# RohanVKashyap/resolution-pde

Measured on AMD Instinct MI355X. Metric: training samples/sec, FFNO2D NS 256^2, higher is better.
Workload: dtype f32; 1 GPU; FFNO2D(1,1,width=64,n_layers=4,n_modes=20,factor=4,ff_weight_norm,n_ff_layers=3,layer_norm,dropout=0.1) train step on [B,1,256,256] Gaussian random fields (BASELINE configs[2]); batch_per_gpu=32, global_batch=32, optimizer=AdamW lr=1e-3 (rpde.optim.FlatAdamW: torch.optim.AdamW's rule, one kernel), parallelism=single, grad_bucket_bytes=6828576, target=input advanced by a fixed spectral filter (utils/synthetic.py:advance)

## Files before the change

resolution-pde_amd/csrc/ff_bwd_split.hip:

```cpp
#include "ff_bwd_split.h"
#include "ff_fused.h"
#include "h2.h"
#include "pointwise.h"
#include "wgrad_h2.h"

namespace rpde {

constexpr int FS_WAVES = 8;
constexpr int FS_MAX_GRID = 256;
struct FsA {
  const float* g; const float* z3; const float* d2;
  float* dz3; float* du2; float* dzb;
  const char* wimg; const float* consts;
  const float* gamma; const float* beta;
  float* part;
  long P; int layer_norm; float eps; int post_act;
  DropCfg drop2;
  int ntiles;
};

constexpr int FA_DZBUF = 0;
constexpr int FA_VEC = FA_DZBUF + 16384;
constexpr int FA_ACC = FA_VEC + 512;
constexpr int FA_INFO = FA_ACC + 7168;
constexpr int FA_LDS = FA_INFO + 256;

__global__ __launch_bounds__(64 * FS_WAVES, 2) void k_ffs_adjoint(const FsA A0) {
  __shared__ __attribute__((aligned(16))) char smem[FA_LDS];
  FsA A = A0;
  A.drop2 = drop_resolve(A0.drop2);
  const int tid = threadIdx.x, l = tid & 63, w = tid >> 6, g = l >> 4, li = l & 15;
  f16x8 w3h[2][2], w3l[2][2];
  {
    const char* base = A.wimg + (long)w * FF3_WAVE_IMG + l * 16;
#pragma unroll
    for (int f = 0; f < 4; ++f) {
      w3h[f >> 1][f & 1] = *reinterpret_cast<const f16x8*>(base + f * 2048);
      w3l[f >> 1][f & 1] = *reinterpret_cast<const f16x8*>(base + f * 2048 + 1024);
    }
    float* vecw = reinterpret_cast<float*>(smem + FA_VEC);
    float* accw = reinterpret_cast<float*>(smem + FA_ACC);
    for (int i = tid; i < 128; i += 64 * FS_WAVES) vecw[i] = i < 64 ? (A.gamma ? A.gamma[i] : 1.f) : (A.beta ? A.beta[i - 64] : 0.f);
    for (int i = tid; i < 1792; i += 64 * FS_WAVES) accw[i] = 0.f;
  }
  const float* const vec = reinterpret_cast<const float*>(smem + FA_VEC);
  float* const acc_db2 = reinterpret_cast<float*>(smem + FA_ACC);
  float* const acc_db3 = acc_db2 + 256;
  float* const acc_dg = acc_db2 + 768;
  float* const acc_dbt = acc_db2 + 1280;
  float* const info = reinterpret_cast<float*>(smem + FA_INFO);
  const float winv3 = A.consts[2];
  const int q3 = l >> 4, feat = 4 * li;

  float4 g4n = make_float4(0.f, 0.f, 0.f, 0.f), z4n = g4n, d2n[4];
  auto issue = [&](int tile) {
    const long p = min((long)tile * 32 + 4 * w + q3, A.P - 1);
    g4n = *reinterpret_cast<const float4*>(A.g + p * 64 + feat);
    z4n = *reinterpret_cast<const float4*>(A.z3 + p * 64 + feat);
#pragma unroll
    for (int blk = 0; blk < 2; ++blk)
#pragma unroll
      for (int t = 0; t < 2; ++t)
        d2n[blk * 2 + t] = *reinterpret_cast<const float4*>(A.d2 + min((long)tile * 32 + 16 * blk + li, A.P - 1) * 256 + 16 * (2 * w + t) + 4 * g);
  };
#pragma unroll
  for (int i = 0; i < 4; ++i) d2n[i] = make_float4(0.f, 0.f, 0.f, 0.f);
  if ((int)blockIdx.x < A.ntiles) issue(blockIdx.x);
  lds_barrier();

  int par = 0;
  for (int tile = blockIdx.x; tile < A.ntiles; tile += gridDim.x, par ^= 1) {
    const int next_tile = tile + gridDim.x;
    const long p0 = (long)tile * 32;
    const int ptl = 4 * w + q3;
    const long pt3 = p0 + ptl;
    const bool live3 = pt3 < A.P;
    const long off3 = min(pt3, A.P - 1) * 64 + feat;
    const float4 g4 = g4n, z4 = z4n;
    float4 dq[4];
#pragma unroll
    for (int i = 0; i < 4; ++i) dq[i] = d2n[i];
    if (next_tile < A.ntiles) issue(next_tile);

    float s4[4] = {1.f, 1.f, 1.f, 1.f};
    if (A.drop2.on()) drop_scale4(A.drop2, (uint64_t)(pt3 * 64 + feat), s4);
    const float tz[4] = {z4.x * s4[0], z4.y * s4[1], z4.z * s4[2], z4.w * s4[3]};
    float gy[4] = {g4.x, g4.y, g4.z, g4.w};
    if (!live3) { gy[0] = gy[1] = gy[2] = gy[3] = 0.f; }
    float dz[4], dzb;
    float dgm[4] = {0.f, 0.f, 0.f, 0.f}, dbt[4] = {0.f, 0.f, 0.f, 0.f};
    if (A.layer_norm) {
      const float mean = row_all16<false>((tz[0] + tz[1]) + (tz[2] + tz[3])) * (1.f / 64.f);
      const float m2 = row_all16<false>((tz[0] - mean) * (tz[0] - mean) + (tz[1] - mean) * (tz[1] - mean) +
                                        (tz[2] - mean) * (tz[2] - mean) + (tz[3] - mean) * (tz[3] - mean));
      const float rstd = rsqrtf(m2 * (1.f / 64.f) + A.eps);
      const float4 gm = *reinterpret_cast<const float4*>(vec + feat);
      const float4 bt = *reinterpret_cast<const float4*>(vec + 64 + feat);
      const float gmv[4] = {gm.x, gm.y, gm.z, gm.w}, btv[4] = {bt.x, bt.y, bt.z, bt.w};
      float xh[4], dxh[4], s1 = 0.f, s2 = 0.f, am = 0.f;
#pragma unroll
      for (int k = 0; k < 4; ++k) {
        xh[k] = (tz[k] - mean) * rstd;
        float dy = gy[k];
        if (A.post_act) dy *= dact_f(A.post_act, xh[k] * gmv[k] + btv[k]);
        dgm[k] = dy * xh[k];
        dbt[k] = dy;
        dxh[k] = dy * gmv[k];
        s1 += dxh[k];
        s2 += dxh[k] * xh[k];
        am = fmaxf(am, fabsf(dxh[k]));
      }
      const float S1 = row_all16<false>(s1) * (1.f / 64.f), S2 = row_all16<false>(s2) * (1.f / 64.f);
      const float AM = row_all16<true>(am);
#pragma unroll
      for (int k = 0; k < 4; ++k) dz[k] = rstd * (dxh[k] - S1 - xh[k] * S2) * s4[k];
      dzb = rstd * (AM + fabsf(S1) + 8.f * fabsf(S2)) * A.drop2.scale;
    } else {
      float am = 0.f;
#pragma unroll
      for (int k = 0; k < 4; ++k) { dz[k] = gy[k] * dact_f(A.post_act, tz[k]) * s4[k]; am = fmaxf(am, fabsf(dz[k])); }
      dzb = row_all16<true>(am);
    }
    if (live3) *reinterpret_cast<float4*>(A.dz3 + off3) = make_float4(dz[0], dz[1], dz[2], dz[3]);
    {
      float b[4];
#pragma unroll
      for (int k = 0; k < 4; ++k) {
        b[k] = live3 ? dz[k] : 0.f;
        b[k] += lane_xor16(b[k]); b[k] += lane_xor32(b[k]);
        if (A.layer_norm) {
          dgm[k] += lane_xor16(dgm[k]); dgm[k] += lane_xor32(dgm[k]);
          dbt[k] += lane_xor16(dbt[k]); dbt[k] += lane_xor32(dbt[k]);
        }
      }
      if (q3 == 0) {
        float4* a3 = reinterpret_cast<float4*>(acc_db3 + w * 64 + feat);
        float4 v3 = *a3;
        v3.x += b[0]; v3.y += b[1]; v3.z += b[2]; v3.w += b[3];
        *a3 = v3;
        if (A.layer_norm) {
          float4* ag = reinterpret_cast<float4*>(acc_dg + w * 64 + feat);
          float4* ab = reinterpret_cast<float4*>(acc_dbt + w * 64 + feat);
          float4 vg = *ag, vb = *ab;
          vg.x += dgm[0]; vg.y += dgm[1]; vg.z += dgm[2]; vg.w += dgm[3];
          vb.x += dbt[0]; vb.y += dbt[1]; vb.z += dbt[2]; vb.w += dbt[3];
          *ag = vg;
          *ab = vb;
        }
      }
    }
    {
      float sdz, sdzi;
      h2_scale(dzb, 0, sdz, sdzi);
      uint2 hi, lo;
      h2_split4(dz[0] * sdz, dz[1] * sdz, dz[2] * sdz, dz[3] * sdz, hi, lo);
      const int ksz = li >> 3, cz = li & 3;
      char* dst = smem + FA_DZBUF + par * 8192 + (((ptl >> 4) * 2 + ksz) * 2) * 1024 + (cz * 16 + ((ptl & 15) ^ cz ^ (4 * ksz))) * 16 +
                  ((li >> 2) & 1) * 8;
      *reinterpret_cast<uint2*>(dst) = hi;
      *reinterpret_cast<uint2*>(dst + 1024) = lo;
      if (li == 0) {
        info[par * 32 + ptl] = dzb;
        if (live3) A.dzb[pt3] = dzb;
      }
    }
    lds_barrier();

    float bsum[8] = {0.f, 0.f, 0.f, 0.f, 0.f, 0.f, 0.f, 0.f};
#pragma unroll
    for (int blk = 0; blk < 2; ++blk) {
      const int zu = (l & 48) | ((l & 15) ^ (l >> 4));
      const char* zb = smem + FA_DZBUF + par * 8192 + (blk * 2) * 2048;
      const f16x8 zh0 = *reinterpret_cast<const f16x8*>(zb + zu * 16), zl0 = *reinterpret_cast<const f16x8*>(zb + 1024 + zu * 16);
      const f16x8 zh1 = *reinterpret_cast<const f16x8*>(zb + 2048 + (zu ^ 4) * 16), zl1 = *reinterpret_cast<const f16x8*>(zb + 3072 + (zu ^ 4) * 16);
      const long pt = p0 + 16 * blk + li;
      float sz, inv_a;
      h2_scale(info[par * 32 + blk * 16 + li], 0, sz, inv_a);
      inv_a *= winv3;
#pragma unroll
      for (int t = 0; t < 2; ++t) {
        f32x4v acc = {0.f, 0.f, 0.f, 0.f};
        acc = h2_mfma32(w3h[t][0], w3l[t][0], zh0, zl0, acc);
        acc = h2_mfma32(w3h[t][1], w3l[t][1], zh1, zl1, acc);
        const int hid = 16 * (2 * w + t) + 4 * g;
        const float4 d = dq[blk * 2 + t];
        float u[4] = {acc[0] * inv_a * d.x, acc[1] * inv_a * d.y, acc[2] * inv_a * d.z, acc[3] * inv_a * d.w};
#pragma unroll
        for (int r = 0; r < 4; ++r) pin(u[r]);
        if (pt < A.P) {
          *reinterpret_cast<float4*>(A.du2 + pt * 256 + hid) = make_float4(u[0], u[1], u[2], u[3]);
#pragma unroll
          for (int r = 0; r < 4; ++r) bsum[4 * t + r] += u[r];
        }
      }
    }
#pragma unroll
    for (int i = 0; i < 8; ++i) bsum[i] = row_sum15(bsum[i]);
    if (li == 15) {
#pragma unroll
      for (int i = 0; i < 8; ++i) acc_db2[16 * (2 * w + (i >> 2)) + 4 * g + (i & 3)] += bsum[i];
    }
  }
  lds_barrier();
  {
    float* part = A.part + (long)blockIdx.x * FF3_PART;
    for (int i = 256 + tid; i < FF3_PART; i += 64 * FS_WAVES) {
      float v;
      if (i < 512) v = acc_db2[i - 256];
      else {
        const float* a8 = acc_db3 + ((i - 512) >> 6) * 512 + ((i - 512) & 63);
        v = 0.f;
#pragma unroll
        for (int ww = 0; ww < FS_WAVES; ++ww) v += a8[ww * 64];
      }
      part[i] = v;
    }
  }
}

struct FsB {
  const float* du2; const float* d1; const float* x; const float* dzb; const float* w1;
  float* gx; float* slabs; float* part;
  const char* wimg; const float* consts;
  long P; float dmax; int ntiles;
};

constexpr int FL_PANEL = 8192;
constexpr int FL_DUBUF = 0;
constexpr int FL_PAN = FL_DUBUF + 32768;
constexpr int FL_X = FL_PAN + 4 * FL_PANEL;
constexpr int FL_W1 = FL_X + FL_PANEL;
constexpr int FL_LDS = FL_W1 + 65536;

__global__ __launch_bounds__(64 * FS_WAVES, 2) void k_ffs_layer1(const FsB A) {
  __shared__ __attribute__((aligned(16))) char smem[FL_LDS];
  __shared__ int einfo[FS_WAVES];
  __shared__ float xmax[FS_WAVES];
  __shared__ float wmax[FS_WAVES];
  __shared__ float acc_db1[256];
  const int tid = threadIdx.x, l = tid & 63, w = tid >> 6, g = l >> 4, li = l & 15;
  f16x8 w2h[2][8], w2l[2][8];
  {
    const char* base = A.wimg + (long)w * FF3_WAVE_IMG + l * 16;
#pragma unroll
    for (int f = 0; f < 16; ++f) {
      w2h[f >> 3][f & 7] = *reinterpret_cast<const f16x8*>(base + (4 + f) * 2048);
      w2l[f >> 3][f & 7] = *reinterpret_cast<const f16x8*>(base + (4 + f) * 2048 + 1024);
    }
  }
  if (tid < 256) acc_db1[tid] = 0.f;
  char* const wfrag = smem + FL_W1;
  float w_inv = 1.f;
  {
    constexpr int NF = 8 * 4 * 64 / (64 * FS_WAVES);
    float wv[NF][8];
    float m = 0.f;
#pragma unroll
    for (int r = 0; r < NF; ++r) {
      const int c = tid + r * 64 * FS_WAVES, fl = c & 63, nt = (c >> 6) & 3, ks = c >> 8;
#pragma unroll
      for (int j = 0; j < 8; ++j) {
        wv[r][j] = A.w1[(long)(32 * ks + 8 * (fl >> 4) + j) * 64 + 16 * nt + (fl & 15)];
        m = fmaxf(m, fabsf(wv[r][j]));
      }
    }
    m = wave_max(m);
    if (l == 0) wmax[w] = m;
    __syncthreads();
    m = 0.f;
#pragma unroll
    for (int i = 0; i < FS_WAVES; ++i) m = fmaxf(m, wmax[i]);
    float w_scale;
    h2_scale(m, 0, w_scale, w_inv);
#pragma unroll
    for (int r = 0; r < NF; ++r) {
      const int c = tid + r * 64 * FS_WAVES, fl = c & 63, nt = (c >> 6) & 3, ks = c >> 8;
      uint2 h0, l0, h1, l1;
      h2_split4(wv[r][0] * w_scale, wv[r][1] * w_scale, wv[r][2] * w_scale, wv[r][3] * w_scale, h0, l0);
      h2_split4(wv[r][4] * w_scale, wv[r][5] * w_scale, wv[r][6] * w_scale, wv[r][7] * w_scale, h1, l1);
      char* d = wfrag + (ks * 4 + nt) * 2048 + fl * 16;
      *reinterpret_cast<uint4*>(d) = make_uint4(h0.x, h0.y, h1.x, h1.y);
      *reinterpret_cast<uint4*>(d + 1024) = make_uint4(l0.x, l0.y, l1.x, l1.y);
    }
  }
  const float winv2 = A.consts[1], c3t = A.consts[3];

  const int xrow = tid >> 4, xc = tid & 15;
  float4 du2r[4], d1r[4], xr;
  float bzr[2];
  const unsigned cb = 32 * w + 4 * g;
  auto load_du2 = [&](int tile) {
    const long t0 = (long)tile * 32;
    const int rmax = (int)min(31L, A.P - 1 - t0);
    const float* __restrict__ src = A.du2 + t0 * 256;
    const float* __restrict__ bz = A.dzb + t0;
#pragma unroll
    for (int blk = 0; blk < 2; ++blk) {
      const unsigned r = (unsigned)min(16 * blk + li, rmax);
      bzr[blk] = bz[r];
#pragma unroll
      for (int t = 0; t < 2; ++t) du2r[blk * 2 + t] = *reinterpret_cast<const float4*>(src + (r * 256u + cb + 16u * t));
    }
  };
  auto load_d1 = [&](int tile) {
    const long t0 = (long)tile * 32;
    const int rmax = (int)min(31L, A.P - 1 - t0);
    const float* __restrict__ src = A.d1 + t0 * 256;
#pragma unroll
    for (int blk = 0; blk < 2; ++blk) {
      const unsigned r = (unsigned)min(16 * blk + li, rmax);
#pragma unroll
      for (int t = 0; t < 2; ++t) d1r[blk * 2 + t] = *reinterpret_cast<const float4*>(src + (r * 256u + cb + 16u * t));
    }
  };
  auto load_x = [&](int tile) {
    const long t0 = (long)tile * 32;
    const float* __restrict__ src = A.x + t0 * 64;
    xr = t0 + xrow < A.P ? *reinterpret_cast<const float4*>(src + (unsigned)(xrow * 64 + 4 * xc)) : make_float4(0.f, 0.f, 0.f, 0.f);
  };

  const int wm = w >> 1, wn = w & 1;
  typedef s16x4v __attribute__((address_space(3))) * lds_tr;
  f32x4v gw[4][2];
#pragma unroll
  for (int i = 0; i < 4; ++i)
#pragma unroll
    for (int j = 0; j < 2; ++j) gw[i][j] = (f32x4v){0.f, 0.f, 0.f, 0.f};
  int ea_used[2] = {15, 15}, eb_used = 15;
  int e_run = 15, e_x = 15;
  const int dg_mt = w & 1, dg_nt = w >> 1;

  if ((int)blockIdx.x < A.ntiles) { load_du2(blockIdx.x); load_d1(blockIdx.x); load_x(blockIdx.x); }
  lds_barrier();

  for (int tile = blockIdx.x; tile < A.ntiles; tile += gridDim.x) {
    const int next_tile = tile + gridDim.x;
    const bool has_next = next_tile < A.ntiles;
    const long p0 = (long)tile * 32;
    float inv_b[2];
#pragma unroll
    for (int blk = 0; blk < 2; ++blk) {
      float s_du2, ai;
      h2_scale(c3t * bzr[blk] * A.dmax, 0, s_du2, ai);
      inv_b[blk] = ai * winv2;
      const float4 a = du2r[blk * 2], b = du2r[blk * 2 + 1];
      const float hv[8] = {a.x * s_du2, a.y * s_du2, a.z * s_du2, a.w * s_du2, b.x * s_du2, b.y * s_du2, b.z * s_du2, b.w * s_du2};
      h2_put_frag(smem + FL_DUBUF + ((blk * 8 + w) * 2) * 1024 + l * 16, hv);
    }
    {
      float m = fmaxf(fmaxf(fabsf(xr.x), fabsf(xr.y)), fmaxf(fabsf(xr.z), fabsf(xr.w)));
      m = wave_max(m);
      if (l == 0) xmax[w] = m;
    }
    lds_barrier();

    float u[4][4];
    float bsum[8] = {0.f, 0.f, 0.f, 0.f, 0.f, 0.f, 0.f, 0.f};
    {
      f32x4v acc[2][2];
#pragma unroll
      for (int blk = 0; blk < 2; ++blk) {
        acc[blk][0] = (f32x4v){0.f, 0.f, 0.f, 0.f}; acc[blk][1] = (f32x4v){0.f, 0.f, 0.f, 0.f};
#pragma unroll
        for (int kap = 0; kap < 8; ++kap) {
          const char* hb = smem + FL_DUBUF + ((blk * 8 + kap) * 2) * 1024 + l * 16;
          const f16x8 bh = *reinterpret_cast<const f16x8*>(hb), bl = *reinterpret_cast<const f16x8*>(hb + 1024);
          acc[blk][0] = h2_mfma32(w2h[0][kap], w2l[0][kap], bh, bl, acc[blk][0]);
          acc[blk][1] = h2_mfma32(w2h[1][kap], w2l[1][kap], bh, bl, acc[blk][1]);
        }
      }
#pragma unroll
      for (int blk = 0; blk < 2; ++blk) {
        const bool live = p0 + 16 * blk + li < A.P;
#pragma unroll
        for (int t = 0; t < 2; ++t) {
          const float4 d4 = d1r[blk * 2 + t];
          const float d[4] = {d4.x, d4.y, d4.z, d4.w};
          float* v = u[blk * 2 + t];
          float s[4];
#pragma unroll
          for (int r = 0; r < 4; ++r) { s[r] = acc[blk][t][r] * inv_b[blk]; v[r] = s[r] * d[r]; }
          if (live) {
#pragma unroll
            for (int r = 0; r < 4; ++r) bsum[4 * t + r] = __builtin_fmaf(s[r], d[r], bsum[4 * t + r]);
          } else {
            v[0] = v[1] = v[2] = v[3] = 0.f;
          }
        }
      }
    }
    if (has_next) { load_du2(next_tile); load_d1(next_tile); }
#pragma unroll
    for (int i = 0; i < 8; ++i) bsum[i] = row_sum15(bsum[i]);
    if (li == 15) {
#pragma unroll
      for (int i = 0; i < 8; ++i) acc_db1[16 * (2 * w + (i >> 2)) + 4 * g + (i & 3)] += bsum[i];
    }
    {
      float m = 0.f;
#pragma unroll
      for (int i = 0; i < 4; ++i) m = fmaxf(fmaxf(m, fmaxf(fabsf(u[i][0]), fabsf(u[i][1]))), fmaxf(fabsf(u[i][2]), fabsf(u[i][3])));
      m = wave_max(m);
      e_run = max(e_run, (int)(__float_as_uint(m) >> 23) & 0xff);
      e_run = min(e_run, 254);
      const float scale = __uint_as_float((unsigned)(268 - e_run) << 23);
      char* const dst = smem + FL_PAN + (w >> 1) * FL_PANEL;
#pragma unroll
      for (int blk = 0; blk < 2; ++blk)
#pragma unroll
        for (int t = 0; t < 2; ++t) {
          const float* v = u[blk * 2 + t];
          uint2 hi, lo;
          h2_split4(v[0] * scale, v[1] * scale, v[2] * scale, v[3] * scale, hi, lo);
          const int off = stage_off(16 * blk + li, (w & 1) * 8 + 4 * t + g);
          *reinterpret_cast<uint2*>(dst + off) = hi;
          *reinterpret_cast<uint2*>(dst + 4096 + off) = lo;
        }
      if (l == 0) einfo[w] = e_run;
    }
    {
      float m = 0.f;
#pragma unroll
      for (int i = 0; i < FS_WAVES; ++i) m = fmaxf(m, xmax[i]);
      e_x = max(e_x, (int)(__float_as_uint(m) >> 23) & 0xff);
      e_x = min(e_x, 254);
      const float scale = __uint_as_float((unsigned)(268 - e_x) << 23);
      uint2 hi, lo;
      h2_split4(xr.x * scale, xr.y * scale, xr.z * scale, xr.w * scale, hi, lo);
      const int off = stage_off(xrow, xc);
      *reinterpret_cast<uint2*>(smem + FL_X + off) = hi;
      *reinterpret_cast<uint2*>(smem + FL_X + 4096 + off) = lo;
    }
    if (has_next) load_x(next_tile);
    lds_barrier();

    int lc = l;
    asm volatile("" : "+v"(lc));
    const int gc = lc >> 4, lic = lc & 15;
    {
      const int q = lic >> 2, pp = lic & 3;
      const int tsw = ((q >> 1) & 1) | ((gc & 1) << 1);
      const int trow = (8 * gc + q) * 128 + pp * 8;
      auto frag = [&](const char* panel, int tile, f16x8& hi, f16x8& lo) {
        const char* t = panel + trow + ((tile ^ tsw) << 5);
        union { struct { s16x4v a, b; } h; f16x8 v; } uh, ul;
        uh.h.a = __builtin_amdgcn_ds_read_tr16_b64_v4i16((lds_tr)(t));
        uh.h.b = __builtin_amdgcn_ds_read_tr16_b64_v4i16((lds_tr)(t + 512));
        ul.h.a = __builtin_amdgcn_ds_read_tr16_b64_v4i16((lds_tr)(t + 4096));
        ul.h.b = __builtin_amdgcn_ds_read_tr16_b64_v4i16((lds_tr)(t + 4096 + 512));
        hi = uh.v; lo = ul.v;
      };
      const int eb = __builtin_amdgcn_readfirstlane(e_x);
#pragma unroll
      for (int k = 0; k < 2; ++k) {
        const int ea = __builtin_amdgcn_readfirstlane(einfo[2 * wm + k]);
        if (ea + eb != ea_used[k] + eb_used) {
          const int d = (ea_used[k] + eb_used) - (ea + eb);
          const float f = d > -126 ? __uint_as_float((unsigned)(127 + d) << 23) : 0.f;
#pragma unroll
          for (int j = 0; j < 2; ++j) { gw[2 * k][j] *= f; gw[2 * k + 1][j] *= f; }
        }
        ea_used[k] = ea;
      }
      eb_used = eb;
      f16x8 bh[2], bl[2];
#pragma unroll
      for (int j = 0; j < 2; ++j) frag(smem + FL_X, 2 * wn + j, bh[j], bl[j]);
#pragma unroll
      for (int i = 0; i < 4; ++i) {
        f16x8 ah, al;
        frag(smem + FL_PAN + wm * FL_PANEL, i, ah, al);
#pragma unroll
        for (int j = 0; j < 2; ++j) gw[i][j] = h2_mfma32(ah, al, bh[j], bl[j], gw[i][j]);
      }
    }
    {
      f32x4v tot = (f32x4v){0.f, 0.f, 0.f, 0.f};
      const int row = 16 * dg_mt + lic;
#pragma unroll
      for (int hp = 0; hp < 8; ++hp) {
        const char* pa_ = smem + FL_PAN + (hp >> 1) * FL_PANEL + stage_off(row, 2 * (4 * (hp & 1) + gc));
        const f16x8 ah = *reinterpret_cast<const f16x8*>(pa_), al = *reinterpret_cast<const f16x8*>(pa_ + 4096);
        const char* wb = wfrag + (hp * 4 + dg_nt) * 2048 + lc * 16;
        const f16x8 bh = *reinterpret_cast<const f16x8*>(wb), bl = *reinterpret_cast<const f16x8*>(wb + 1024);
        const f32x4v part = h2_mfma32(ah, al, bh, bl, (f32x4v){0.f, 0.f, 0.f, 0.f});
        const int ek = __builtin_amdgcn_readfirstlane(einfo[hp]);
        const float fk = __uint_as_float((unsigned)(ek - 14) << 23) * w_inv;
        tot += part * fk;
      }
      float t0 = tot[0], t1 = tot[1], t2 = tot[2], t3 = tot[3];
      quad_transpose(t0, t1, t2, t3);
      const int rq = 16 * dg_mt + 4 * gc + (lic & 3);
      if (p0 + rq < A.P) *reinterpret_cast<float4*>(A.gx + p0 * 64 + (unsigned)(rq * 64 + 16 * dg_nt + 4 * (lic >> 2))) = make_float4(t0, t1, t2, t3);
    }
  }

  const float fb = __uint_as_float((unsigned)(eb_used - 14) << 23);
  float* __restrict__ out = A.slabs + (long)blockIdx.x * 256 * 64;
  const unsigned o0 = (unsigned)((wm * 64 + 4 * g) * 64 + wn * 32 + li);
#pragma unroll
  for (int i = 0; i < 4; ++i) {
    const float fa = __uint_as_float((unsigned)(ea_used[i >> 1] - 14) << 23);
#pragma unroll
    for (int j = 0; j < 2; ++j)
#pragma unroll
      for (int r = 0; r < 4; ++r) out[o0 + (unsigned)((16 * i + r) * 64 + 16 * j)] = gw[i][j][r] * fa * fb;
  }
  lds_barrier();
  if (tid < 256) A.part[(long)blockIdx.x * FF3_PART + tid] = acc_db1[tid];
}

bool ff_bwd_split_ok(long P, int hid, int dim) { return !switch_off("RPDE_FF_BWD_SPLIT") && wgrad_h2_dgrad_ok(P, hid, dim); }

int ff_bwd_split_launch(const rpde_ff_params* p, const float* const* ds, const float* z_last, const float* grad_out,
                        const float* x, float* dz3, float* du2, float* dzb, float* gx, float* slabs, float* gw1, float* part,
                        int* grid_out, long P, void* fimg, hipStream_t st, FoldJobs* folds) {
  RPDE_CHECK_ARG(ff_bwd_split_ok(P, p->dim * p->factor, p->dim) && ds && ds[0] && ds[1] && gx && gw1 && slabs,
                 "ff_bwd_split: unsupported call");
  const char* img;
  const float* consts;
  RPDE_TRY(ff3_fused_bwd_prepare(p, fimg, &img, &consts, st));
  const int ntiles = (int)((P + 31) / 32);
  int cus;
  RPDE_HIP(cu_count(&cus));
  int grid = cus < FS_MAX_GRID ? cus : FS_MAX_GRID;
  if (ntiles < grid) grid = ntiles;
  const DropCfg drop2 = make_drop(p->dropout_p, layer_seed(p->seed, 2), p->seed_epoch);

  FsA a;
  memset(&a, 0, sizeof(a));
  a.g = grad_out; a.z3 = z_last; a.d2 = ds[1];
  a.dz3 = dz3; a.du2 = du2; a.dzb = dzb;
  a.wimg = img; a.consts = consts; a.gamma = p->ln_gamma; a.beta = p->ln_beta; a.part = part;
  a.P = P; a.layer_norm = p->layer_norm; a.eps = p->ln_eps; a.post_act = p->post_act;
  a.drop2 = drop2; a.ntiles = ntiles;
  hipLaunchKernelGGL(k_ffs_adjoint, dim3(grid), dim3(64 * FS_WAVES), 0, st, a);
  RPDE_LAUNCH_CHECK();

  FsB b;
  memset(&b, 0, sizeof(b));
  b.du2 = du2; b.d1 = ds[0]; b.x = x; b.dzb = dzb; b.w1 = p->weights[0];
  b.gx = gx; b.slabs = slabs; b.part = part;
  b.wimg = img; b.consts = consts;
  b.P = P; b.dmax = 1.13f * drop2.scale;
  b.ntiles = ntiles;
  hipLaunchKernelGGL(k_ffs_layer1, dim3(grid), dim3(64 * FS_WAVES), 0, st, b);
  RPDE_LAUNCH_CHECK();
  *grid_out = grid;
  const int hid = p->dim * p->factor;
  if (folds && folds->add(slabs, gw1, hid * p->dim, grid, (long)hid * p->dim)) return RPDE_OK;
  return reduce_slabs(slabs, gw1, (long)hid * p->dim, grid, (long)hid * p->dim, 1.f, 0, st);
}

}
```

Before: 1046 samples/s.

## Restructure FF layer-1 backward pipeline: deeper prefetch, parked W2 fragments, priority split

Reworks the k_ffs_layer1 tile loop so du2 is staged into LDS one tile ahead and fetched two tiles ahead, while d1 and the x maximum for the next tile are loaded at the end of the current iteration. Loads are clamped to the last tile, which removes the has_next branches. Part of the W2 low-half fragments is parked in extra LDS to reduce register pressure, and the dgrad loop double-buffers its LDS fragment reads. Upper waves get a raised scheduling priority. Optional timestamp instrumentation and a profiling script are added behind RPDE_STAMPS. The cost is more LDS, which may affect occupancy at two blocks per CU, plus some redundant clamped loads.

Measured after the change: 1058 samples/s, median of 6. 1.01x the previous value.

```diff
diff --git a/profiles/ffs_layer1_stamps.py b/profiles/ffs_layer1_stamps.py
--- /dev/null
+++ b/profiles/ffs_layer1_stamps.py
@@ -0,0 +1,40 @@
+#!/usr/bin/env python3
+import ctypes as C
+import os
+import sys
+
+REPO = os.path.dirname(os.path.dirname(os.path.abspath(__file__)))
+for p in (REPO, os.path.join(REPO, "resolution-pde_amd")):
+    sys.path.insert(0, p)
+import numpy as np
+import torch
+from rpde import _lib
+from models.custom_layer import FeedForward
+
+lib = _lib.load()
+torch.manual_seed(0)
+ff = FeedForward(64, 4, n_layers=3, layer_norm=True, dropout=0.1).to("cuda")
+x = torch.randn(32, 256, 256, 64, device="cuda").requires_grad_(True)
+res, g = torch.randn_like(x), torch.randn_like(x)
+for _ in range(3):
+    ff(x, residual=res).backward(g)
+torch.cuda.synchronize()
+buf = (C.c_ulonglong * (3 * 64))()
+lib.rpde_debug_ffl_stamps.argtypes = [C.c_void_p]
+_lib.check(lib.rpde_debug_ffl_stamps(buf), "stamps")
+t = np.array(buf, dtype=np.uint64).reshape(3, 8, 8).astype(np.int64)
+names = ["top", "barrier 1 passed", "products + scaling done", "panels written, x requested", "barrier 2 passed",
+         "next du2 staged + requested", "gW1 done", "gx done"]
+for wi, wn in enumerate(("wave 0", "wave 3", "wave 6")):
+    print(wn)
+    for ti in range(7):
+        row = t[wi, ti]
+        print("   tile", ti + 5, " ".join(f"{names[i]}:+{int(row[i] - row[0])}" for i in range(1, 8)),
+              f" | tile period {int(t[wi, ti + 1, 0] - row[0])}")
+per = (t[:, 1:, 0] - t[:, :-1, 0]).astype(np.float64)
+seg = np.diff(np.concatenate([t[:, :7, :], t[:, 1:, :1]], axis=2), axis=2).astype(np.float64)
+print("mean share of the tile period, waves 0 / 3 / 6:")
+for i in range(8):
+    what = f"{names[i]} -> {names[i + 1] if i < 7 else 'x maximum, next top'}"
+    print(f"   {what:64s}", " ".join(f"{100 * (seg[wv, :, i] / per[wv]).mean():5.1f}%" for wv in range(3)))
+print("mean tile period:", " ".join(f"{per[wv].mean():.0f}" for wv in range(3)))
diff --git a/resolution-pde_amd/csrc/ff_bwd_split.hip b/resolution-pde_amd/csrc/ff_bwd_split.hip
--- a/resolution-pde_amd/csrc/ff_bwd_split.hip
+++ b/resolution-pde_amd/csrc/ff_bwd_split.hip
@@ -230,7 +230,15 @@
 constexpr int FL_PAN = FL_DUBUF + 32768;
 constexpr int FL_X = FL_PAN + 4 * FL_PANEL;
 constexpr int FL_W1 = FL_X + FL_PANEL;
-constexpr int FL_LDS = FL_W1 + 65536;
+constexpr int FL_W2L = FL_W1 + 65536;
+constexpr int FL_LDS = FL_W2L + 16384;
+#ifdef RPDE_STAMPS
+__device__ unsigned long long g_flstamps[3 * 64];
+#define FLSTAMP(i) do { if (stamp_on && stamp_t >= 0 && stamp_t < 8) g_flstamps[stamp_w * 64 + stamp_t * 8 + (i)] = __builtin_amdgcn_s_memtime(); } while (0)
+#else
+#define FLSTAMP(i) do { } while (0)
+#endif
+constexpr int FL_PARKED = 7;
 
 __global__ __launch_bounds__(64 * FS_WAVES, 2) void k_ffs_layer1(const FsB A) {
   __shared__ __attribute__((aligned(16))) char smem[FL_LDS];
@@ -239,13 +247,16 @@
   __shared__ float wmax[FS_WAVES];
   __shared__ float acc_db1[256];
   const int tid = threadIdx.x, l = tid & 63, w = tid >> 6, g = l >> 4, li = l & 15;
-  f16x8 w2h[2][8], w2l[2][8];
+  f16x8 w2h[2][8], w2l[2][FL_PARKED];
+  char* const parked = smem + FL_W2L + w * 2048 + l * 16;
   {
     const char* base = A.wimg + (long)w * FF3_WAVE_IMG + l * 16;
 #pragma unroll
     for (int f = 0; f < 16; ++f) {
       w2h[f >> 3][f & 7] = *reinterpret_cast<const f16x8*>(base + (4 + f) * 2048);
-      w2l[f >> 3][f & 7] = *reinterpret_cast<const f16x8*>(base + (4 + f) * 2048 + 1024);
+      const f16x8 lo = *reinterpret_cast<const f16x8*>(base + (4 + f) * 2048 + 1024);
+      if ((f & 7) < FL_PARKED) w2l[f >> 3][f & 7] = lo;
+      else *reinterpret_cast<f16x8*>(parked + (f >> 3) * 1024) = lo;
     }
   }
   if (tid < 256) acc_db1[tid] = 0.f;
@@ -289,8 +300,9 @@
   float4 du2r[4], d1r[4], xr;
   float bzr[2];
   const unsigned cb = 32 * w + 4 * g;
+  const int last_tile = A.ntiles - 1;
   auto load_du2 = [&](int tile) {
-    const long t0 = (long)tile * 32;
+    const long t0 = (long)min(tile, last_tile) * 32;
     const int rmax = (int)min(31L, A.P - 1 - t0);
     const float* __restrict__ src = A.du2 + t0 * 256;
     const float* __restrict__ bz = A.dzb + t0;
@@ -303,7 +315,7 @@
     }
   };
   auto load_d1 = [&](int tile) {
-    const long t0 = (long)tile * 32;
+    const long t0 = (long)min(tile, last_tile) * 32;
     const int rmax = (int)min(31L, A.P - 1 - t0);
     const float* __restrict__ src = A.d1 + t0 * 256;
 #pragma unroll
@@ -314,9 +326,13 @@
     }
   };
   auto load_x = [&](int tile) {
-    const long t0 = (long)tile * 32;
+    const long t0 = (long)min(tile, last_tile) * 32;
+    const int rmax = (int)min(31L, A.P - 1 - t0);
     const float* __restrict__ src = A.x + t0 * 64;
-    xr = t0 + xrow < A.P ? *reinterpret_cast<const float4*>(src + (unsigned)(xrow * 64 + 4 * xc)) : make_float4(0.f, 0.f, 0.f, 0.f);
+    xr = *reinterpret_cast<const float4*>(src + (unsigned)(min(xrow, rmax) * 64 + 4 * xc));
+  };
+  auto x_of = [&](int tile) {
+    return (long)tile * 32 + xrow < A.P ? xr : make_float4(0.f, 0.f, 0.f, 0.f);
   };
 
   const int wm = w >> 1, wn = w & 1;
@@ -330,14 +346,8 @@
   int e_run = 15, e_x = 15;
   const int dg_mt = w & 1, dg_nt = w >> 1;
 
-  if ((int)blockIdx.x < A.ntiles) { load_du2(blockIdx.x); load_d1(blockIdx.x); load_x(blockIdx.x); }
-  lds_barrier();
-
-  for (int tile = blockIdx.x; tile < A.ntiles; tile += gridDim.x) {
-    const int next_tile = tile + gridDim.x;
-    const bool has_next = next_tile < A.ntiles;
-    const long p0 = (long)tile * 32;
-    float inv_b[2];
+  float inv_b[2];
+  auto stage_du2 = [&]() {
 #pragma unroll
     for (int blk = 0; blk < 2; ++blk) {
       float s_du2, ai;
@@ -347,12 +357,30 @@
       const float hv[8] = {a.x * s_du2, a.y * s_du2, a.z * s_du2, a.w * s_du2, b.x * s_du2, b.y * s_du2, b.z * s_du2, b.w * s_du2};
       h2_put_frag(smem + FL_DUBUF + ((blk * 8 + w) * 2) * 1024 + l * 16, hv);
     }
-    {
-      float m = fmaxf(fmaxf(fabsf(xr.x), fabsf(xr.y)), fmaxf(fabsf(xr.z), fabsf(xr.w)));
-      m = wave_max(m);
-      if (l == 0) xmax[w] = m;
-    }
+  };
+  auto stage_xmax = [&](int tile) {
+    const float4 xv = x_of(tile);
+    float m = fmaxf(fmaxf(fabsf(xv.x), fabsf(xv.y)), fmaxf(fabsf(xv.z), fabsf(xv.w)));
+    m = wave_max(m);
+    if (l == 0) xmax[w] = m;
+  };
+
+  load_du2(blockIdx.x); load_d1(blockIdx.x); load_x(blockIdx.x);
+  lds_barrier();
+  stage_du2(); stage_xmax(blockIdx.x);
+  load_du2(blockIdx.x + gridDim.x);
+  if (__builtin_amdgcn_readfirstlane(w) >= 4) __builtin_amdgcn_s_setprio(1);
+#ifdef RPDE_STAMPS
+  const bool stamp_on = blockIdx.x == 100 && l == 0 && (w == 0 || w == 3 || w == 6);
+  const int stamp_w = w == 0 ? 0 : (w == 3 ? 1 : 2);
+  int stamp_t = -4;
+#endif
+  for (int tile = blockIdx.x; tile < A.ntiles; tile += gridDim.x) {
+    const int next_tile = tile + gridDim.x;
+    const long p0 = (long)tile * 32;
+    FLSTAMP(0);
     lds_barrier();
+    FLSTAMP(1);
 
     float u[4][4];
     float bsum[8] = {0.f, 0.f, 0.f, 0.f, 0.f, 0.f, 0.f, 0.f};
@@ -365,8 +393,14 @@
         for (int kap = 0; kap < 8; ++kap) {
           const char* hb = smem + FL_DUBUF + ((blk * 8 + kap) * 2) * 1024 + l * 16;
           const f16x8 bh = *reinterpret_cast<const f16x8*>(hb), bl = *reinterpret_cast<const f16x8*>(hb + 1024);
-          acc[blk][0] = h2_mfma32(w2h[0][kap], w2l[0][kap], bh, bl, acc[blk][0]);
-          acc[blk][1] = h2_mfma32(w2h[1][kap], w2l[1][kap], bh, bl, acc[blk][1]);
+          if (kap < FL_PARKED) {
+            acc[blk][0] = h2_mfma32(w2h[0][kap], w2l[0][kap], bh, bl, acc[blk][0]);
+            acc[blk][1] = h2_mfma32(w2h[1][kap], w2l[1][kap], bh, bl, acc[blk][1]);
+          } else {
+            const f16x8 l0 = *reinterpret_cast<const f16x8*>(parked), l1 = *reinterpret_cast<const f16x8*>(parked + 1024);
+            acc[blk][0] = h2_mfma32(w2h[0][kap], l0, bh, bl, acc[blk][0]);
+            acc[blk][1] = h2_mfma32(w2h[1][kap], l1, bh, bl, acc[blk][1]);
+          }
         }
       }
 #pragma unroll
@@ -389,7 +423,7 @@
         }
       }
     }
-    if (has_next) { load_du2(next_tile); load_d1(next_tile); }
+    FLSTAMP(2);
 #pragma unroll
     for (int i = 0; i < 8; ++i) bsum[i] = row_sum15(bsum[i]);
     if (li == 15) {
@@ -426,13 +460,20 @@
       e_x = min(e_x, 254);
       const float scale = __uint_as_float((unsigned)(268 - e_x) << 23);
       uint2 hi, lo;
-      h2_split4(xr.x * scale, xr.y * scale, xr.z * scale, xr.w * scale, hi, lo);
+      const float4 xv = x_of(tile);
+      h2_split4(xv.x * scale, xv.y * scale, xv.z * scale, xv.w * scale, hi, lo);
       const int off = stage_off(xrow, xc);
       *reinterpret_cast<uint2*>(smem + FL_X + off) = hi;
       *reinterpret_cast<uint2*>(smem + FL_X + 4096 + off) = lo;
     }
-    if (has_next) load_x(next_tile);
+    load_x(next_tile);
+    FLSTAMP(3);
     lds_barrier();
+    FLSTAMP(4);
+
+    stage_du2();
+    load_du2(next_tile + gridDim.x);
+    FLSTAMP(5);
 
     int lc = l;
     asm volatile("" : "+v"(lc));
@@ -474,16 +515,22 @@
         for (int j = 0; j < 2; ++j) gw[i][j] = h2_mfma32(ah, al, bh[j], bl[j], gw[i][j]);
       }
     }
+    FLSTAMP(6);
     {
       f32x4v tot = (f32x4v){0.f, 0.f, 0.f, 0.f};
       const int row = 16 * dg_mt + lic;
+      f16x8 ah[2], al[2], bh[2], bl[2];
+      auto frags = [&](int hp) {
+        const char* pa_ = smem + FL_PAN + (hp >> 1) * FL_PANEL + stage_off(row, 2 * (4 * (hp & 1) + gc));
+        ah[hp & 1] = *reinterpret_cast<const f16x8*>(pa_); al[hp & 1] = *reinterpret_cast<const f16x8*>(pa_ + 4096);
+        const char* wb = wfrag + (hp * 4 + dg_nt) * 2048 + lc * 16;
+        bh[hp & 1] = *reinterpret_cast<const f16x8*>(wb); bl[hp & 1] = *reinterpret_cast<const f16x8*>(wb + 1024);
+      };
+      frags(0);
 #pragma unroll
       for (int hp = 0; hp < 8; ++hp) {
-        const char* pa_ = smem + FL_PAN + (hp >> 1) * FL_PANEL + stage_off(row, 2 * (4 * (hp & 1) + gc));
-        const f16x8 ah = *reinterpret_cast<const f16x8*>(pa_), al = *reinterpret_cast<const f16x8*>(pa_ + 4096);
-        const char* wb = wfrag + (hp * 4 + dg_nt) * 2048 + lc * 16;
-        const f16x8 bh = *reinterpret_cast<const f16x8*>(wb), bl = *reinterpret_cast<const f16x8*>(wb + 1024);
-        const f32x4v part = h2_mfma32(ah, al, bh, bl, (f32x4v){0.f, 0.f, 0.f, 0.f});
+        if (hp + 1 < 8) frags(hp + 1);
+        const f32x4v part = h2_mfma32(ah[hp & 1], al[hp & 1], bh[hp & 1], bl[hp & 1], (f32x4v){0.f, 0.f, 0.f, 0.f});
         const int ek = __builtin_amdgcn_readfirstlane(einfo[hp]);
         const float fk = __uint_as_float((unsigned)(ek - 14) << 23) * w_inv;
         tot += part * fk;
@@ -493,6 +540,12 @@
       const int rq = 16 * dg_mt + 4 * gc + (lic & 3);
       if (p0 + rq < A.P) *reinterpret_cast<float4*>(A.gx + p0 * 64 + (unsigned)(rq * 64 + 16 * dg_nt + 4 * (lic >> 2))) = make_float4(t0, t1, t2, t3);
     }
+    FLSTAMP(7);
+    load_d1(next_tile);
+    stage_xmax(next_tile);
+#ifdef RPDE_STAMPS
+    ++stamp_t;
+#endif
   }
 
   const float fb = __uint_as_float((unsigned)(eb_used - 14) << 23);
@@ -553,3 +606,11 @@
 }
 
 }
+
+#ifdef RPDE_STAMPS
+extern "C" int rpde_debug_ffl_stamps(unsigned long long* host_out) {
+  RPDE_HIP(hipDeviceSynchronize());
+  RPDE_HIP(hipMemcpyFromSymbol(host_out, HIP_SYMBOL(rpde::g_flstamps), sizeof(unsigned long long) * 3 * 64));
+  return RPDE_OK;
+}
+#endif
```
